# Visual-Behavior/detr-tensorflow

Measured on AMD Instinct MI355X. Metric: images/sec training step, DETR-R50 800x1333 bs=8/GPU, higher is better.
Workload: dtype bf16

## Files before the change

### detr-tensorflow_amd/csrc/conv_f32.hip

```cpp
#include "gemm_core.h"
#include "gemm_bf16_core.h"
#include "conv_args.h"
#include "conv_halo.h"
#include "conv_halo_dma.h"
namespace detr {

template <int BM, bool DGRAD, int DIL = 1>
struct LoaderConvA {
    static constexpr int NV = BM / 64;
    BufSrc src;
    int n_[NV], h_[NV], w_[NV];
    bool ok[NV];
    int kq, tid;

    __device__ __forceinline__ void init(const ConvArgs &a, int m0, int tid_) {
        src.init(a.src, (long long)a.N * a.Hs * a.Ws * a.Cs);
        tid = tid_;
        kq = (tid & 3) * 4;
#pragma unroll
        for (int i = 0; i < NV; ++i) {
            const int m = m0 + (tid >> 2) + 64 * i;
            ok[i] = m < a.M;
            const int mm = ok[i] ? m : 0;
            int wd, hd;
// ... 567 lines not shown
        if (++it_chunk == chunks) {
            it_chunk = 0;
            if (++it_ho == a.Ho) {
                it_ho = 0;
                ++it_n;
            }
        }
#pragma unroll
        for (int i = 0; i < NRD; ++i) {
            const int v = S16 ? 2 * tid : tid + 256 * i;
            const int j = 4 * (v >> 6) + ((v >> 2) & 3);
            const int col = 16 * ((v >> 4) & 3) + 4 * (v & 3);
            const bool ok = live && wo0 + j < a.Wo;
            const unsigned off = ((unsigned)((n * a.Ho + ho) * a.Wo + wo0 + j) * (unsigned)a.Co + (unsigned)(co0 + col)) * (S16 ? 2u : 4u);
            if constexpr (S16) rd[i] = ds.ld16(ok ? off : BUF_OOB);
            else rd[i] = ds.ld4(ok ? off : BUF_OOB);
        }
#pragma unroll
        for (int i = 0; i < NRX; ++i) {
            const int v = tid + 256 * i;
            const int pp = S16 ? v >> 3 : v >> 4, c4 = S16 ? 2 * (v & 7) : v & 15;
            const int kh = pp / PC, c = pp - kh * PC;
            const int hi = STR * ho - 1 + kh, wi = STR * wo0 - 1 + c;
            const bool ok = live && pp < NPP && hi >= 0 && hi < a.Hi && wi >= 0 && wi < a.Wi;
            const unsigned off = ((unsigned)((n * a.Hi + hi) * a.Wi + wi) * (unsigned)a.Ci + (unsigned)(ci0 + 4 * c4)) * (S16 ? 2u : 4u);
            if constexpr (S16) rx[i] = xs.ld16(ok ? off : BUF_OOB);
            else rx[i] = xs.ld4(ok ? off : BUF_OOB);
        }
    };
    auto store_unit = [&](int buf, const Reg (&rx)[NRX], const Reg (&rd)[NRD]) {
#pragma unroll
        for (int i = 0; i < NRD; ++i) {
            if constexpr (S16) *reinterpret_cast<uint4 *>(&sm.D[buf][tid * 8]) = rd[i];
            else *reinterpret_cast<uint2 *>(&sm.D[buf][(tid + 256 * i) * 4]) = make_uint2(pack_bf16(rd[i].x, rd[i].y), pack_bf16(rd[i].z, rd[i].w));
        }
#pragma unroll
        for (int i = 0; i < NRX; ++i) {
            const int v = tid + 256 * i;
            const int pp = S16 ? v >> 3 : v >> 4, c4 = S16 ? 2 * (v & 7) : v & 15;
            if (pp < NPP) {
                const int kh = pp / PC, c = WG::slot(pp - kh * PC);
                const int o = kh * WF_ROW + ((c >> 2) * 4 + (c4 >> 2)) * 64 + (((c & 3) + (c4 >> 2)) & 3) * 16 + (c4 & 3) * 4;
                if constexpr (S16) *reinterpret_cast<uint4 *>(&sm.X[buf][o]) = rx[i];
                else *reinterpret_cast<uint2 *>(&sm.X[buf][o]) = make_uint2(pack_bf16(rx[i].x, rx[i].y), pack_bf16(rx[i].z, rx[i].w));
            }
        }
    };
    typedef __attribute__((address_space(3))) s16x4 lds_s16x4;
    typedef short s16x8 __attribute__((ext_vector_type(8)));
    const int g = lane >> 4, t16 = lane & 15;
    int xo[2][3][2], dofs[2];
#pragma unroll
    for (int s2 = 0; s2 < 2; ++s2) {
        const int cib = 2 * wm + (g & 1);
        const int jbase = 16 * s2 + 8 * (g >> 1) + (t16 >> 2);
#pragma unroll
        for (int kw = 0; kw < 3; ++kw)
#pragma unroll
            for (int h = 0; h < 2; ++h) {
                const int c = STR == 1 ? jbase + kw + 4 * h : (kw & 1) * 33 + jbase + (kw >> 1) + 4 * h;
                xo[s2][kw][h] = ((c >> 2) * 4 + cib) * 64 + (((c & 3) + cib) & 3) * 16 + (t16 & 3) * 4;
            }
        dofs[s2] = ((4 * s2 + 2 * (g >> 1)) * 4 + 2 * wn + (g & 1)) * 64 + t16 * 4;
    }
    load_unit(u_begin, rx0, rd0);
    store_unit(0, rx0, rd0);
    load_unit(u_begin + 1, rx0, rd0);
    load_unit(u_begin + 2, rx1, rd1);
    lds_barrier();
    auto iter = [&](const int u, const int cur, Reg (&rpx)[NRX], Reg (&rpd)[NRD]) {
        store_unit(cur ^ 1, rpx, rpd);
        load_unit(u + 3, rpx, rpd);
        const unsigned short *X = sm.X[cur];
        const unsigned short *D = sm.D[cur];
#pragma unroll
        for (int s2 = 0; s2 < 2; ++s2) {
            const s16x4 blo = __builtin_amdgcn_ds_read_tr16_b64_v4i16((lds_s16x4 *)(D + dofs[s2]));
            const s16x4 bhi = __builtin_amdgcn_ds_read_tr16_b64_v4i16((lds_s16x4 *)(D + dofs[s2] + 4 * 64));
            const bf16x8 bfrag = __builtin_bit_cast(bf16x8, (s16x8)__builtin_shufflevector(blo, bhi, 0, 1, 2, 3, 4, 5, 6, 7));
#pragma unroll
            for (int kh = 0; kh < 3; ++kh)
#pragma unroll
                for (int kw = 0; kw < 3; ++kw) {
                    const s16x4 lo = __builtin_amdgcn_ds_read_tr16_b64_v4i16((lds_s16x4 *)(X + xo[s2][kw][0] + kh * WF_ROW));
                    const s16x4 hi = __builtin_amdgcn_ds_read_tr16_b64_v4i16((lds_s16x4 *)(X + xo[s2][kw][1] + kh * WF_ROW));
                    const bf16x8 afrag = __builtin_bit_cast(bf16x8, (s16x8)__builtin_shufflevector(lo, hi, 0, 1, 2, 3, 4, 5, 6, 7));
                    acc[kh * 3 + kw] = __builtin_amdgcn_mfma_f32_32x32x16_bf16(afrag, bfrag, acc[kh * 3 + kw], 0, 0, 0);
                }
        }
        lds_barrier();
    };
    {
        int u = u_begin;
        for (; u + 2 <= u_end; u += 2) {
            iter(u, 0, rx0, rd0);
            iter(u + 1, 1, rx1, rd1);
        }
        if (u < u_end) iter(u, 0, rx0, rd0);
    }
    if (a.slab_ts) {
#pragma unroll
        for (int t = 0; t < 9; ++t) {
            f32x16 one[1][1];
            one[0][0] = acc[t];
            float *slab = a.dw + (long long)blockIdx.z * a.part_stride + ((long long)(t * a.tiles_m + tm) * a.tiles_n + tn) * (64 * 64);
            store_slab_ts<64, 64, 2, 2>(one, slab, wave, lane);
        }
        return;
    }
    __syncthreads();
#pragma unroll
    for (int t = 0; t < 9; ++t) {
        f32x16 one[1][1];
        one[0][0] = acc[t];
        float *dw = a.dw + (long long)t * a.Ci * a.Co + (long long)blockIdx.z * a.part_stride;
        epilogue<64, 64, 2, 2, false>(one, reinterpret_cast<float *>(smem_raw), dw, a.Co, a.Ci, a.Co, ci0, co0, wm, wn, lane, wave, a.e, t == 0);
    }
}

typedef void (*ConvKernel)(ConvArgs);
typedef void (*WgradKernel)(ConvWgradArgs);

static void launch_conv_tiles(ConvKernel kernel, int bm, int bn, const ConvArgs &a0, hipStream_t s) {
    ConvArgs a = a0;
    a.tiles_m = cdiv(a.M, bm);
    a.tiles_n = cdiv(a.Cd, bn);
    dim3 grid((unsigned)(a.tiles_m * a.tiles_n)), block(GEMM_THREADS);
    hipLaunchKernelGGL(kernel, grid, block, 0, s, a);
}

template <int BM, int BN, int DIL, bool W16, bool X16>
static ConvKernel conv_bf16c_dir(bool dgrad) {
    return dgrad ? conv3x3_bf16c_kernel<BM, BN, 2, 2, true, W16, X16, DIL> : conv3x3_bf16c_kernel<BM, BN, 2, 2, false, W16, X16, DIL>;
}
template <int BM, int BN, int DIL>
static ConvKernel conv_bf16c_for(const ConvArgs &a, bool dgrad) {
    if (a.w16 && a.x16) return conv_bf16c_dir<BM, BN, DIL, true, true>(dgrad);
    if (a.w16) return conv_bf16c_dir<BM, BN, DIL, true, false>(dgrad);
    if (a.x16) return conv_bf16c_dir<BM, BN, DIL, false, true>(dgrad);
    return conv_bf16c_dir<BM, BN, DIL, false, false>(dgrad);
}

static bool x3_form(const ConvArgs &a) { return a.Cs % 32 == 0 && tune(T_X3_CONV) != 2 && (!a.par_on || tune(T_X3_CONV) == 1); }

template <int BM, int BN>
static void launch_conv(const ConvArgs &a, bool dgrad, hipStream_t s, bool split3 = false) {
    ConvKernel k = dgrad ? conv3x3_kernel<BM, BN, 2, 2, true> : conv3x3_kernel<BM, BN, 2, 2, false>;
    if constexpr (BM == BN) {
        if (split3 && x3_form(a)) k = dgrad ? conv3x3_x3_kernel<BM, BN, true> : conv3x3_x3_kernel<BM, BN, false>;
        else if (split3) k = dgrad ? conv3x3_kernel<BM, BN, 2, 2, true, true> : conv3x3_kernel<BM, BN, 2, 2, false, true>;
    }
    launch_conv_tiles(k, BM, BN, a, s);
}

static int wgrad_split_plan(int M, int tiles, int split, int &rps) {
    if (split <= 0) {
        split = cdiv(1536, tiles * 9);
        const int max_split = cdiv(M, 256);
        if (split > max_split) split = max_split;
        if (split < 1) split = 1;
    }
    rps = cdiv(M, split);
    rps = ((rps + BF_BK - 1) / BF_BK) * BF_BK;
    return cdiv(M, rps);
}
static int wgrad_x3_split(int M, int tiles, int bm) {
    const int rounds = tune(T_X3_WG_ROUNDS) > 0 ? tune(T_X3_WG_ROUNDS) : 2;
    const int slots = bm >= 128 ? 512 : 1024;
    int split = (rounds * slots) / (tiles * 9);
    const int max_split = cdiv(M, 256);
    if (split > max_split) split = max_split;
    return split < 1 ? 1 : split;
}
static int wgrad_fused_split_plan(int units, int tiles, int split, int &ups) {
    if (split <= 0) {
        int wgs = tune(T_WGRAD_FUSED_WGS);
        if (wgs <= 2) wgs = 512;
        split = cdiv(wgs, tiles);
    }
    if (split > units) split = units;
    if (split < 1) split = 1;
    ups = cdiv(units, split);
    return cdiv(units, ups);
}

struct WgradPlan {
    bool fused;
    int tile;
    int split;
    int per_split;
    long long bytes;
};

static WgradPlan wgrad_plan(int N, int Ho, int Wo, int Ci, int Co, int stride, int pad, bool s16, int compute, int dil, int split) {
    WgradPlan p;
    const bool bf = compute == 1 && Ci % 32 == 0 && Co % 32 == 0;
    const int fmode = tune(T_WGRAD_FUSED);
    const bool s_ok = stride == 1 || (stride == 2 && s16 && fmode != 3 && (fmode == 4 || (Ci <= 128 && Co <= 128)));
    p.fused = dil == 1 && bf && s_ok && pad == 1 && Ci % 64 == 0 && Co % 64 == 0 && fmode != 2;
    if (p.fused) {
        p.tile = 64;
        p.split = wgrad_fused_split_plan(N * Ho * cdiv(Wo, 32), (Ci / 64) * (Co / 64), split, p.per_split);
    } else {
        const int wforce = (bf || dil != 1) ? 0 : tune(T_WGRAD_TILE);
        p.tile = (wforce == 3) ? 64 : ((wforce == 1 || (Ci >= 128 && Co >= 128)) ? 128 : 64);
        const int M = N * Ho * Wo, tiles = cdiv(Ci, p.tile) * cdiv(Co, p.tile);
        if (compute == 2 && split <= 0 && tune(T_X3_CONV) != 2) split = wgrad_x3_split(M, tiles, p.tile);
        p.split = wgrad_split_plan(M, tiles, split, p.per_split);
    }
    p.bytes = p.split > 1 ? (long long)p.split * 9LL * Ci * Co * 4 : 0;
    return p;
}

template <class Launch>
static void wgrad_run(const ConvWgradArgs &a0, const WgradPlan &p, int taps_y, float *ws, long long ws_bytes, hipStream_t s, Launch launch) {
    ConvWgradArgs a = a0;
    a.tiles_m = cdiv(a.Ci, p.tile);
    a.tiles_n = cdiv(a.Co, p.tile);
    a.rows_per_split = p.per_split;
    const long long part = 9LL * a.Ci * a.Co;
    const bool partial = p.split > 1 && ws && aligned16(ws) && ws_bytes >= p.bytes;
    float *dw_final = a.dw;
    const EpiArgs final_e = a.e;
    a.part_stride = 0;
    a.slab_ts = 0;
    const bool ts = partial && a.Ci % p.tile == 0 && a.Co % p.tile == 0 && (!final_e.scale || aligned16(final_e.scale)) &&
                    aligned16(dw_final) && tune(T_SLAB_TS) != 2;
    if (partial) {
        a.dw = ws; a.part_stride = part;
        a.e.alpha = 1.0f;
        a.e.scale = nullptr;
        a.e.atomic = 0;
        a.e.vec = 1;
        a.slab_ts = ts ? 1 : 0;
    } else {
        a.e.atomic = 1;
    }
    launch(a, dim3((unsigned)(a.tiles_m * a.tiles_n), (unsigned)taps_y, (unsigned)p.split));
    if (partial) {
        detr_reduce_desc r = {};
        r.ws = ws; r.splits = p.split; r.part_stride = part; r.rows = 9 * a.Ci; r.cols = a.Co;
        r.C = dw_final; r.ldc = a.Co; r.alpha = final_e.alpha; r.scale = final_e.scale; r.rs_alpha = 1.0f;
        if (ts) { r.ts_bm = r.ts_bn = p.tile; r.ts_tiles_n = a.tiles_n; }
        launch_splitk_reduce(r, s);
    }
}

template <int BT>
static void launch_wgrad(const ConvWgradArgs &a0, const WgradPlan &p, float *ws, long long ws_bytes, hipStream_t s, bool bf16c, bool split3) {
    WgradKernel k;
    if (a0.dil == 2) {
        if (bf16c) k = a0.s16 ? conv3x3_wgrad_bf16c_kernel<BT, BT, 2, 2, true, 2> : conv3x3_wgrad_bf16c_kernel<BT, BT, 2, 2, false, 2>;
        else k = split3 ? conv3x3_wgrad_kernel<BT, BT, 2, 2, true, 2> : conv3x3_wgrad_kernel<BT, BT, 2, 2, false, 2>;
    } else if (bf16c) k = a0.s16 ? conv3x3_wgrad_bf16c_kernel<BT, BT, 2, 2, true> : conv3x3_wgrad_bf16c_kernel<BT, BT, 2, 2, false>;
    else if (split3) k = tune(T_X3_CONV) != 2 ? conv3x3_wgrad_x3_kernel<BT, BT> : conv3x3_wgrad_kernel<BT, BT, 2, 2, true>;
    else k = conv3x3_wgrad_kernel<BT, BT, 2, 2>;
    wgrad_run(a0, p, 9, ws, ws_bytes, s, [&](const ConvWgradArgs &a, dim3 grid) { hipLaunchKernelGGL(k, grid, dim3(GEMM_THREADS), 0, s, a); });
}

static void launch_wgrad_fused(const ConvWgradArgs &a0, const WgradPlan &p, float *ws, long long ws_bytes, hipStream_t s) {
    const int chunks = cdiv(a0.Wo, 32);
    wgrad_run(a0, p, 1, ws, ws_bytes, s, [&](const ConvWgradArgs &a, dim3 grid) {
        const dim3 block(GEMM_THREADS);
        if (a.stride == 2) hipLaunchKernelGGL((conv3x3_wgrad_fused_bf16_kernel<true, 2>), grid, block, 0, s, a, p.per_split, chunks);
        else if (a.s16) hipLaunchKernelGGL(conv3x3_wgrad_fused_bf16_kernel<true>, grid, block, 0, s, a, p.per_split, chunks);
        else hipLaunchKernelGGL(conv3x3_wgrad_fused_bf16_kernel<false>, grid, block, 0, s, a, p.per_split, chunks);
    });
}

static void launch_wgrad_plan(const ConvWgradArgs &a, const WgradPlan &p, float *ws, long long ws_bytes, hipStream_t s, bool bf16c, bool split3) {
    if (p.fused) launch_wgrad_fused(a, p, ws, ws_bytes, s);
    else if (p.tile == 128) launch_wgrad<128>(a, p, ws, ws_bytes, s, bf16c, split3);
    else launch_wgrad<64>(a, p, ws, ws_bytes, s, bf16c, split3);
}

void conv_dilated_tiles(const ConvArgs &a, bool dgrad, int compute, hipStream_t s) {
    ConvKernel k;
    if (compute == 1) k = conv_bf16c_for<64, 64, 2>(a, dgrad);
    else if (compute == 2) k = dgrad ? conv3x3_kernel<64, 64, 2, 2, true, true, 2> : conv3x3_kernel<64, 64, 2, 2, false, true, 2>;
    else k = dgrad ? conv3x3_kernel<64, 64, 2, 2, true, false, 2> : conv3x3_kernel<64, 64, 2, 2, false, false, 2>;
    launch_conv_tiles(k, 64, 64, a, s);
}

static WgradPlan conv_dilated_wgrad_plan(int N, int H, int W, int Ci, int Co, bool s16, int compute, int split) {
    return wgrad_plan(N, H, W, Ci, Co, 1, 2, s16, compute, 2, split);
}

void conv_dilated_wgrad_tiles(const ConvWgradArgs &a, int compute, int split, float *ws, long long ws_bytes, hipStream_t s) {
    launch_wgrad_plan(a, conv_dilated_wgrad_plan(a.N, a.Ho, a.Wo, a.Ci, a.Co, a.s16, compute, split), ws, ws_bytes, s, compute == 1, compute == 2);
}

int conv_dilated_wgrad_splits(int N, int H, int W, int Ci, int Co, int compute, int split) {
    return conv_dilated_wgrad_plan(N, H, W, Ci, Co, false, compute, split).split;
}

}

using namespace detr;

static WgradPlan wgrad_plan(const detr_conv3x3_desc *d) {
    return wgrad_plan(d->N, d->Ho, d->Wo, d->Ci, d->Co, d->stride, d->pad, d->x_dtype == 1 && d->w_dtype == 1, d->compute, 1, d->split);
}

static bool halo_eligible(const detr_conv3x3_desc *d, const ConvArgs &a, const EpiArgs &e, bool dgrad_classes) {
    if (!(d->compute == 1 && d->pad == 1 && a.w16 && a.x16 && e.c16 && a.Cs % 32 == 0 && a.Cd % 64 == 0 && a.Cd <= 512 &&
          (!d->mask || e.m16) && !d->residual && !d->scale && d->alpha == 1.0f && tune(T_CONV_HALO) != 2)) return false;
    if (dgrad_classes) return d->stride == 2 && !d->bias && d->act == 0 && tune(T_DGRAD_S2_CLASSES) != 3;
    return d->stride == 1 && (d->act == 0 || d->act == 1);
}

extern "C" int64_t detr_hip_workspace_bytes_conv3x3(const detr_conv3x3_desc *d, int32_t mode) {
    if (!d || d->N <= 0 || d->Ci <= 0 || d->Co <= 0) return -1;
    if (mode != 2) return 0;
    return wgrad_plan(d).bytes;
}

extern "C" int detr_hip_conv3x3_f32(const detr_conv3x3_desc *d, int32_t mode, void *stream) {
    DETR_REQUIRE(d != nullptr, "conv3x3: null descriptor");
    DETR_REQUIRE(mode >= 0 && mode <= 2, "conv3x3: bad mode %d", mode);
    DETR_REQUIRE(d->stride == 1 || d->stride == 2, "conv3x3: stride %d unsupported", d->stride);
    DETR_REQUIRE(d->Ci % 16 == 0 && d->Co % 16 == 0, "conv3x3: Ci=%d Co=%d must be multiples of 16", d->Ci, d->Co);
    DETR_REQUIRE(d->Ho == (d->Hi + 2 * d->pad - 3) / d->stride + 1 && d->Wo == (d->Wi + 2 * d->pad - 3) / d->stride + 1,
                 "conv3x3: output %dx%d inconsistent with input %dx%d pad %d stride %d", d->Ho, d->Wo, d->Hi, d->Wi,
                 d->pad, d->stride);
    DETR_REQUIRE(d->x && d->w && d->y, "conv3x3: null operand");
    DETR_REQUIRE(aligned16(d->x) && aligned16(d->w) && aligned16(d->y), "conv3x3: operands must be 16-byte aligned");
    DETR_REQUIRE((long long)d->N * d->Hi * d->Wi * d->Ci * 4 <= BUF_MAX_BYTES &&
                     (long long)d->N * d->Ho * d->Wo * d->Co * 4 <= BUF_MAX_BYTES,
                 "conv3x3: a tensor spans more than 4 GB (32-bit buffer offsets)");
    hipStream_t s = (hipStream_t)stream;
    EpiArgs e;
    e.alpha = d->alpha;
    e.scale = d->scale;
    e.bias = d->bias;
    e.residual = d->residual;
    e.mask = d->mask;
    e.act = d->act;
    e.atomic = 0;
    e.drop_scale = 0.0f; e.drop_thresh = 0; e.drop_seed = 0;
    const bool bits_in = d->mask && d->m_dtype == 2, bits_out = mode == 0 && d->maskbits_out != nullptr;
    e.vec = (!d->scale || aligned16(d->scale)) && (!d->bias || aligned16(d->bias)) &&
            (!d->residual || aligned16(d->residual)) && (!d->mask || bits_in || aligned16(d->mask));
    e.c16 = (mode != 2 && d->y_dtype == 1); e.r16 = d->r_dtype == 1;
    e.m16 = (d->m_dtype == 1 || d->m_dtype == 2) ? d->m_dtype : 0;
    if (mode == 2) {
        DETR_REQUIRE(!d->bias && !d->residual && !d->mask && d->act == 0, "conv3x3 wgrad: only scale/alpha epilogue");
        ConvWgradArgs a;
        a.N = d->N; a.Hi = d->Hi; a.Wi = d->Wi; a.Ci = d->Ci; a.Ho = d->Ho; a.Wo = d->Wo; a.Co = d->Co;
        a.stride = d->stride; a.pad = d->pad;
        a.x = d->x; a.dy = d->w; a.dw = d->y;
        a.M = d->N * d->Ho * d->Wo;
        a.s16 = (d->x_dtype == 1);
        DETR_REQUIRE(d->x_dtype == d->w_dtype && d->y_dtype == 0, "conv3x3 wgrad: x and dy must share their storage type, dw is fp32");
        DETR_REQUIRE(!a.s16 || (d->compute == 1 && d->Ci % 32 == 0 && d->Co % 32 == 0), "conv3x3 wgrad: bf16 tensors need compute = bf16");
        e.atomic = 1; e.ldr = 0; e.ldmask = 0;
        a.e = e;
        const bool bf = d->compute == 1 && d->Ci % 32 == 0 && d->Co % 32 == 0;
        const WgradPlan p = wgrad_plan(d);
        launch_wgrad_plan(a, p, d->workspace, d->workspace_bytes, s, bf, !bf && d->compute == 2);
        DETR_LAUNCH_CHECK(p.fused ? "conv3x3 wgrad bf16 (fused taps)" : (bf ? "conv3x3 wgrad bf16" : "conv3x3 wgrad"));
        return 0;
    }
    ConvArgs a;
    a.N = d->N; a.stride = d->stride; a.pad = d->pad; a.Ci = d->Ci; a.Co = d->Co;
    a.w = d->w; a.src = d->x; a.dst = d->y;
    if (mode == 0) {
        a.Hs = d->Hi; a.Ws = d->Wi; a.Cs = d->Ci;
        a.Hd = d->Ho; a.Wd = d->Wo; a.Cd = d->Co;
    } else {
        a.Hs = d->Ho; a.Ws = d->Wo; a.Cs = d->Co;
        a.Hd = d->Hi; a.Wd = d->Wi; a.Cd = d->Ci;
    }
    a.M = d->N * a.Hd * a.Wd;
    e.ldr = a.Cd;
    e.ldmask = bits_in ? a.Cd / 8 : a.Cd;
    e.mbits_out = bits_out ? d->maskbits_out : nullptr;
    e.ld_mbits_out = a.Cd / 8;
    e.wide16 = e.c16 && e.vec && (!d->residual || e.r16) && (!d->mask || e.m16) && (tune(T_EPI_WIDE) != 2 || bits_in || bits_out);
    DETR_REQUIRE(!(bits_in || bits_out) || (d->compute == 1 && e.wide16), "conv3x3: bit-packed masks need bf16 x / y / residual tensors (compute = bf16)");
    a.e = e;
    a.w16 = (d->w_dtype == 1);
    a.x16 = (d->x_dtype == 1);
    DETR_REQUIRE((d->x_dtype == 0 && d->y_dtype == 0 && d->r_dtype == 0 && d->m_dtype == 0) || (d->compute == 1 && d->Ci % 32 == 0 && d->Co % 32 == 0),
                 "conv3x3: bf16 tensors need compute = bf16 and channel counts %% 32 == 0");
    DETR_REQUIRE(d->w_dtype == 0 || (d->w_dtype == 1 && d->compute == 1 && mode != 2 && d->Ci % 32 == 0 && d->Co % 32 == 0),
                 "conv3x3: a bf16 kernel tensor needs compute = bf16, mode 0/1 and channel counts %% 32 == 0");
    a.par_on = 0; a.Hp = a.Wp = a.ph = a.pw = a.kh0 = a.kw0 = 0; a.nth = a.ntw = 3;
    a.cls_mix = 0;
    const bool dgrad = mode == 1;
    if (halo_eligible(d, a, e, false)) {
        if (a.Cd >= 128 && a.Cd % 128 == 0 && tune(T_CONV_DMA) != 2 && tune(T_CONV_HALO) != 4) { if (launch_conv_halo_dma(a, dgrad, s)) return -1; }
        else if (a.Cd % 128 == 0) { if (launch_conv_halo<128>(a, dgrad, s)) return -1; }
        else if (launch_conv_halo<64>(a, dgrad, s)) return -1;
        DETR_LAUNCH_CHECK("conv3x3 (halo)");
        return 0;
    }
    const int force = tune(T_CONV_TILE);
    auto launch = [&](const ConvArgs &c) {
        const long long big = (long long)cdiv(c.M, 128) * cdiv(c.Cd, 128);
        if (d->compute == 1 && c.Cs % 32 == 0 && c.Cd % 32 == 0) {
            if (force == 3 || (force == 0 && (c.Cd < 128 || big < 256)))
                launch_conv_tiles(conv_bf16c_for<64, 64, 1>(c, dgrad), 64, 64, c, s);
            else launch_conv_tiles(conv_bf16c_for<128, 128, 1>(c, dgrad), 128, 128, c, s);
        } else if (d->compute == 2) {
            const long long t192 = (long long)cdiv(c.M, 192) * cdiv(c.Cd, 128);
            const bool x3form = x3_form(c);
            if (force == 3 || (force == 0 && (c.Cd < 128 || big < x3_t128_threshold()))) launch_conv<64, 64>(c, dgrad, s, true);
            else if (force == 0 && x3form && tune(T_X3_T192) != 2 && tune(T_X3_T192) != 3 && (tune(T_X3_T192) == 1 || x3_t192_fewer_rounds(big, t192)))
                launch_conv_tiles(dgrad ? conv3x3_x3_kernel<192, 128, true> : conv3x3_x3_kernel<192, 128, false>, 192, 128, c, s);
            else if (force == 0 && x3form && tune(T_X3_T192) != 2 && (tune(T_X3_T192) == 3 || c.Cd == 128 || big <= 384)) 
                launch_conv_tiles(dgrad ? conv3x3_x3_kernel<128, 64, true> : conv3x3_x3_kernel<128, 64, false>, 128, 64, c, s);
            else launch_conv<128, 128>(c, dgrad, s, true);
        } else if (force == 1) launch_conv<128, 128>(c, dgrad, s);
        else if (force == 2) launch_conv<128, 64>(c, dgrad, s);
        else launch_conv<64, 64>(c, dgrad, s);
    };
    if (dgrad && d->stride == 2 && tune(T_DGRAD_S2_CLASSES) != 2) {
        if (halo_eligible(d, a, e, true)) {
            if (a.Cd % 128 == 0) { if (launch_conv_halo_s2classes<128>(a, s)) return -1; }
            else if (launch_conv_halo_s2classes<64>(a, s)) return -1;
            DETR_LAUNCH_CHECK("conv3x3 (halo, stride-2 classes)");
            return 0;
        }
        for (int ph = 0; ph < 2; ++ph)
            for (int pw = 0; pw < 2; ++pw) {
                ConvArgs c = a;
                c.par_on = 1; c.ph = ph; c.pw = pw;
                c.Hp = (a.Hd + 1 - ph) / 2;
                c.Wp = (a.Wd + 1 - pw) / 2;
                c.M = d->N * c.Hp * c.Wp;
                if (c.M <= 0) continue;
                c.kh0 = (ph + d->pad) & 1; c.kw0 = (pw + d->pad) & 1;
                c.nth = c.kh0 ? 1 : 2; c.ntw = c.kw0 ? 1 : 2;
                c.e.remap_w2 = c.Wp; c.e.remap_h2 = c.Hp; c.e.remap_W = a.Wd; c.e.remap_H = a.Hd;
                c.e.remap_ph = ph; c.e.remap_pw = pw;
                launch(c);
            }
    } else {
        launch(a);
    }
    DETR_LAUNCH_CHECK("conv3x3");
    return 0;
}
```

### detr-tensorflow_amd/csrc/conv_halo_dma.h

```cpp
#pragma once
#include "conv_halo.h"
#include "gemm_ring.h"

namespace detr {

constexpr int CHD_TH = 4, CHD_BN = 128, CHD_NB = 3;
constexpr int CHD_PIX = (CHD_TH + 2) * CH_PW;
constexpr int CHD_PP = (CHD_PIX + 15) / 16;
constexpr int CHD_PATCH = CHD_PP * 1024;
constexpr int CHD_BT = CHD_BN * BF_BK * 2;
constexpr int CHD_OFF_B = 2 * CHD_PATCH;
constexpr int CHD_OFF_DUMP = CHD_OFF_B + CHD_NB * CHD_BT;
constexpr int CHD_RING = CHD_OFF_DUMP + 1024;
constexpr int CHD_EPI = StageCfg<CHD_BN, 2>::BYTES;
constexpr int CHD_SMEM = CHD_RING > CHD_EPI ? CHD_RING : CHD_EPI;

template <bool DGRAD, bool LATE, bool DIL = false>
__global__ __launch_bounds__(GEMM_THREADS, 3) void conv3x3_halo_dma_bf16_kernel(ConvArgs a) {
#if defined(__HIP_DEVICE_COMPILE__)
    constexpr int BN = CHD_BN, TH = CHD_TH, NB = CHD_NB;
    using T = TileCfg<TH * CH_TW, BN, 2, 2>;
    extern __shared__ __attribute__((aligned(1024))) char chd_smem[];
    const int tid = threadIdx.x, lane = tid & 63;
    const int wave = __builtin_amdgcn_readfirstlane(tid >> 6);
    const int wm = wave >> 1, wn = wave & 1;
    int id = xcd_remap(blockIdx.x, gridDim.x);
    int ph = 0, pw = 0, Hp = a.Hp, Wp = a.Wp;
    if constexpr (DIL) halo_class_decode(a, id, ph, pw, Hp, Wp);
    const int tn = id % a.tiles_n;
    int t = id / a.tiles_n;
    const int twi = t % Wp;
    t /= Wp;
    const int thi = t % Hp;
    const int n = t / Hp;
    const int h0 = thi * TH, w0 = twi * CH_TW, n0 = tn * BN;
    const int nchunks = a.Cs / BF_BK;
    const unsigned lds0 = ring_lds_addr(chd_smem);

    const unsigned long long src_bytes = (unsigned long long)a.N * a.Hs * a.Ws * a.Cs * 2ull;
    unsigned pvoff[4];
    int plds[4];
#pragma unroll
    for (int i = 0; i < 4; ++i) {
        const int P = wave + 4 * i;
        const int px = 16 * P + (lane >> 2);
        const int pr = px / CH_PW, pc = px - pr * CH_PW;
        const int hq = h0 - 1 + pr, wq = w0 - 1 + pc;
        const int h = DIL ? 2 * hq + ph : hq, w = DIL ? 2 * wq + pw : wq;
        const int c = (lane & 3) ^ ((px >> 2) & 3);
        const bool ok = px < CHD_PIX && hq >= 0 && h < a.Hs && wq >= 0 && w < a.Ws;
        pvoff[i] = ok ? ((unsigned)((n * a.Hs + h) * a.Ws + w) * (unsigned)a.Cs) * 2u + 16u * (unsigned)c : BUF_OOB;
        plds[i] = P < CHD_PP ? P * 1024 : -1;
    }
    auto patch_issue = [&](const int i, const int c) {
        const unsigned left = (c < nchunks) ? (unsigned)(src_bytes - (unsigned long long)c * (BF_BK * 2)) : 0u;
        const u32x4 rs = ring_rsrc(reinterpret_cast<const char *>(a.src) + (long long)c * (BF_BK * 2), left);
        const int base = (c & 1) * CHD_PATCH;
        const int in = plds[i] >= 0 ? -1 : 0;
        const int off = CHD_OFF_DUMP + (in & (base + plds[i] - CHD_OFF_DUMP));
        ring_dma_piece(rs, lds0 + (unsigned)off, pvoff[i]);
    };
    const long long tapstride = (long long)a.Ci * a.Co;
    const unsigned long long w_bytes = 9ull * (unsigned long long)tapstride * 2ull;
    unsigned bvoff[2];
#pragma unroll
    for (int i = 0; i < 2; ++i) {
        const int P = wave + 4 * i;
        if constexpr (!DGRAD) {
            const int kr = lane >> 4, pc = lane & 15;
            const int col = n0 + 8 * (pc ^ (4 * kr));
            bvoff[i] = (col + 8 <= a.Cd) ? (unsigned)(4 * P + kr) * (unsigned)a.Co * 2u + 2u * (unsigned)col : BUF_OOB;
        } else {
            const int r = 16 * P + (lane >> 2);
            const int c = (lane & 3) ^ ((r >> 2) & 3);
            bvoff[i] = (n0 + r < a.Cd) ? (unsigned)(n0 + r) * (unsigned)a.Co * 2u + 16u * (unsigned)c : BUF_OOB;
        }
    }
    auto b_issue = [&](const int c, const int tp, const int slot) {
        const int wt = DGRAD ? 8 - tp : tp;
        const long long e0 = wt * tapstride + (DGRAD ? (long long)c * BF_BK : (long long)c * BF_BK * a.Co);
        const unsigned left = (c < nchunks) ? (unsigned)(w_bytes - (unsigned long long)e0 * 2ull) : 0u;
        const u32x4 rs = ring_rsrc(reinterpret_cast<const char *>(a.w) + e0 * 2, left);
#pragma unroll
        for (int i = 0; i < 2; ++i) ring_dma_piece(rs, lds0 + (unsigned)(CHD_OFF_B + slot * CHD_BT + (wave + 4 * i) * 1024), bvoff[i]);
    };

    f32x16 acc[T::TM][T::TN];
#pragma unroll
    for (int i = 0; i < T::TM; ++i)
#pragma unroll
        for (int j = 0; j < T::TN; ++j)
#pragma unroll
            for (int r = 0; r < 16; ++r) acc[i][j][r] = 0.0f;

    const int l31 = lane & 31, hh = lane >> 5;
    int p0[T::TM];
#pragma unroll
    for (int mi = 0; mi < T::TM; ++mi) p0[mi] = (HaloGeom<TH>::RB * wm + mi) * CH_PW + l31;
    int btr[T::TN], brow[T::TN];
#pragma unroll
    for (int ni = 0; ni < T::TN; ++ni) {
        btr[ni] = ring_tr_lane_off<1>(wn * T::WTN + ni * 32, lane);
        const int r = wn * T::WTN + ni * 32 + l31;
        brow[ni] = r * 64 + 16 * (hh ^ ((r >> 2) & 3));
    }
    bf16x8 fa[2][T::TM], fb[2][T::TN];
    auto read_tap = [&](const int pbuf, const int slot, const int tp) {
        const int toff = (tp / 3) * CH_PW + (tp - 3 * (tp / 3));
        const char *Pb = chd_smem + pbuf * CHD_PATCH;
        const char *Bs = chd_smem + CHD_OFF_B + slot * CHD_BT;
        int pa[T::TM];
#pragma unroll
        for (int mi = 0; mi < T::TM; ++mi) {
            int q = p0[mi];
            asm volatile("" : "+v"(q));
            const int p = q + toff;
            pa[mi] = p * 64 + 16 * (hh ^ ((p >> 2) & 3));
        }
#pragma unroll
        for (int kk = 0; kk < 2; ++kk) {
#pragma unroll
            for (int mi = 0; mi < T::TM; ++mi) fa[kk][mi] = *reinterpret_cast<const bf16x8 *>(Pb + (pa[mi] ^ (32 * kk)));
#pragma unroll
            for (int ni = 0; ni < T::TN; ++ni) {
                if constexpr (!DGRAD) fb[kk][ni] = ring_frag_tr<1>(Bs, btr[ni], kk);
                else fb[kk][ni] = *reinterpret_cast<const bf16x8 *>(Bs + (brow[ni] ^ (32 * kk)));
            }
        }
    };
    auto mma_half = [&](const int kk) {
#pragma unroll
        for (int mi = 0; mi < T::TM; ++mi)
#pragma unroll
            for (int ni = 0; ni < T::TN; ++ni) acc[mi][ni] = __builtin_amdgcn_mfma_f32_32x32x16_bf16(fa[kk][mi], fb[kk][ni], acc[mi][ni], 0, 0, 0);
    };

#pragma unroll
    for (int i = 0; i < 4; ++i) patch_issue(i, 0);
    b_issue(0, 0, 0);
    b_issue(0, 1, 1);
    for (int c = 0; c < nchunks; ++c) {
#pragma unroll
        for (int tp = 0; tp < 9; ++tp) {
            constexpr int READS = 2 * T::TM + (DGRAD ? 2 : 4) * T::TN, MF = 2 * T::TM * T::TN;
            if (tp >= 1 && tp <= 4) ring_wait_vmcnt<3>();
            else ring_wait_vmcnt<2>();
            __builtin_amdgcn_s_barrier();
            asm volatile("" ::: "memory");
            auto issue = [&]() {
                int cc = c;
                asm volatile("" : "+s"(cc));
                if (tp < 4) patch_issue(tp, cc + 1);
                b_issue(cc + (tp + 2) / 9, (tp + 2) % 9, (tp + 2) % NB);
            };
            if constexpr (!LATE) {
                issue();
                read_tap(c & 1, tp % NB, tp);
                mma_half(0);
                mma_half(1);
                sgb_ds_read<READS>();
                sgb_mfma_block<MF, 0, 0, 0>();
            } else {
                read_tap(c & 1, tp % NB, tp);
                mma_half(0);
                sgb_ds_read<READS>();
                sgb_mfma_block<MF / 2, 0, 0, 0>();
                __builtin_amdgcn_sched_barrier(0);
                issue();
                __builtin_amdgcn_sched_barrier(0);
                mma_half(1);
            }
            __builtin_amdgcn_sched_barrier(0);
        }
    }
    ring_wait_vmcnt<0>();
    __syncthreads();
    halo_epilogue<BN, TH, DIL>(acc, reinterpret_cast<float *>(chd_smem), reinterpret_cast<unsigned short *>(a.dst), a, n, h0, w0, n0, wm, wn, lane, wave, ph, pw);
#endif
}

static int launch_conv_halo_dma(const ConvArgs &a0, bool dgrad, hipStream_t s) {
    ConvArgs a = a0;
    a.Hp = cdiv(a.Hd, CHD_TH);
    a.Wp = cdiv(a.Wd, CH_TW);
    a.tiles_m = a.N * a.Hp * a.Wp;
    a.tiles_n = cdiv(a.Cd, CHD_BN);
    const bool late = tune(T_CONV_DMA) != 3;
    const int smem = CHD_SMEM;
    const int k = (dgrad ? 1 : 0) + (late ? 2 : 0);
    const void *fns[4] = {reinterpret_cast<const void *>(conv3x3_halo_dma_bf16_kernel<false, false>), reinterpret_cast<const void *>(conv3x3_halo_dma_bf16_kernel<true, false>),
                          reinterpret_cast<const void *>(conv3x3_halo_dma_bf16_kernel<false, true>), reinterpret_cast<const void *>(conv3x3_halo_dma_bf16_kernel<true, true>)};
    static bool reserved[4] = {false, false, false, false};
    if (!reserved[k]) {
        hipError_t err = hipFuncSetAttribute(fns[k], hipFuncAttributeMaxDynamicSharedMemorySize, smem);
        DETR_REQUIRE(err == hipSuccess, "conv3x3 (halo, DMA): cannot reserve %d bytes of LDS: %s", smem, hipGetErrorString(err));
        reserved[k] = true;
    }
    const dim3 grid((unsigned)(a.tiles_m * a.tiles_n)), block(GEMM_THREADS);
    switch (k) {
        case 0: hipLaunchKernelGGL((conv3x3_halo_dma_bf16_kernel<false, false>), grid, block, smem, s, a); break;
        case 1: hipLaunchKernelGGL((conv3x3_halo_dma_bf16_kernel<true, false>), grid, block, smem, s, a); break;
        case 2: hipLaunchKernelGGL((conv3x3_halo_dma_bf16_kernel<false, true>), grid, block, smem, s, a); break;
        default: hipLaunchKernelGGL((conv3x3_halo_dma_bf16_kernel<true, true>), grid, block, smem, s, a); break;
    }
    return 0;
}

static int launch_conv_halo_dma_planes(const ConvArgs &a0, bool dgrad, hipStream_t s) {
    ConvArgs a = a0;
    a.tiles_n = cdiv(a.Cd, CHD_BN);
    halo_class_plan(a, CHD_TH);
    if (a.cls_off[4] <= 0) return 0;
    a.cls_mix = 1;
    const int smem = CHD_SMEM;
    const void *fns[2] = {reinterpret_cast<const void *>(conv3x3_halo_dma_bf16_kernel<false, true, true>), reinterpret_cast<const void *>(conv3x3_halo_dma_bf16_kernel<true, true, true>)};
    static bool reserved[2] = {false, false};
    const int k = dgrad ? 1 : 0;
    if (!reserved[k]) {
        hipError_t err = hipFuncSetAttribute(fns[k], hipFuncAttributeMaxDynamicSharedMemorySize, smem);
        DETR_REQUIRE(err == hipSuccess, "conv3x3 dilated (halo planes, DMA): cannot reserve %d bytes of LDS: %s", smem, hipGetErrorString(err));
        reserved[k] = true;
    }
    const dim3 grid((unsigned)a.cls_off[4]), block(GEMM_THREADS);
    if (dgrad) hipLaunchKernelGGL((conv3x3_halo_dma_bf16_kernel<true, true, true>), grid, block, smem, s, a);
    else hipLaunchKernelGGL((conv3x3_halo_dma_bf16_kernel<false, true, true>), grid, block, smem, s, a);
    return 0;
}

}
```

Baseline: 531.0.

## Add stride-2 forward path to halo DMA conv via four parity-plane patch loads

Extends the DMA-fed halo conv3x3 kernel with a stride-2 forward variant. The input is split into four parity planes loaded into double-buffered LDS patches, and the nine taps are reordered so each plane buffer is reused across the taps that read it. Stride-2 bf16 forward convs in ResNet-50 with Cd%128==0 previously went through the generic implicit-GEMM tile kernel and now take this path. It adds a complex hand-scheduled tap/plane/vmcnt sequence that carries correctness risk, and it also folds the launch helpers into a single templated reserve-and-launch function.

Measured after the change: 533.4, median of 6. Within noise of the previous version (+0.5%).

```diff
diff --git a/detr-tensorflow_amd/csrc/conv_f32.hip b/detr-tensorflow_amd/csrc/conv_f32.hip
--- a/detr-tensorflow_amd/csrc/conv_f32.hip
+++ b/detr-tensorflow_amd/csrc/conv_f32.hip
@@ -893,11 +893,11 @@
     return wgrad_plan(d->N, d->Ho, d->Wo, d->Ci, d->Co, d->stride, d->pad, d->x_dtype == 1 && d->w_dtype == 1, d->compute, 1, d->split);
 }
 
-static bool halo_eligible(const detr_conv3x3_desc *d, const ConvArgs &a, const EpiArgs &e, bool dgrad_classes) {
+static bool halo_eligible(const detr_conv3x3_desc *d, const ConvArgs &a, const EpiArgs &e, bool dgrad_classes, int stride = 1) {
     if (!(d->compute == 1 && d->pad == 1 && a.w16 && a.x16 && e.c16 && a.Cs % 32 == 0 && a.Cd % 64 == 0 && a.Cd <= 512 &&
           (!d->mask || e.m16) && !d->residual && !d->scale && d->alpha == 1.0f && tune(T_CONV_HALO) != 2)) return false;
     if (dgrad_classes) return d->stride == 2 && !d->bias && d->act == 0 && tune(T_DGRAD_S2_CLASSES) != 3;
-    return d->stride == 1 && (d->act == 0 || d->act == 1);
+    return d->stride == stride && (d->act == 0 || d->act == 1);
 }
 
 extern "C" int64_t detr_hip_workspace_bytes_conv3x3(const detr_conv3x3_desc *d, int32_t mode) {
@@ -986,6 +986,11 @@
         DETR_LAUNCH_CHECK("conv3x3 (halo)");
         return 0;
     }
+    if (mode == 0 && halo_eligible(d, a, e, false, 2) && a.Cd % 128 == 0 && tune(T_CONV_DMA) != 2 && tune(T_CONV_DMA) != 4) {
+        if (launch_conv_halo_dma<true>(a, false, s)) return -1;
+        DETR_LAUNCH_CHECK("conv3x3 (halo, stride-2 plane steps)");
+        return 0;
+    }
     const int force = tune(T_CONV_TILE);
     auto launch = [&](const ConvArgs &c) {
         const long long big = (long long)cdiv(c.M, 128) * cdiv(c.Cd, 128);
diff --git a/detr-tensorflow_amd/csrc/conv_halo_dma.h b/detr-tensorflow_amd/csrc/conv_halo_dma.h
--- a/detr-tensorflow_amd/csrc/conv_halo_dma.h
+++ b/detr-tensorflow_amd/csrc/conv_halo_dma.h
@@ -4,21 +4,36 @@
 
 namespace detr {
 
-constexpr int CHD_TH = 4, CHD_BN = 128, CHD_NB = 3;
-constexpr int CHD_PIX = (CHD_TH + 2) * CH_PW;
-constexpr int CHD_PP = (CHD_PIX + 15) / 16;
-constexpr int CHD_PATCH = CHD_PP * 1024;
-constexpr int CHD_BT = CHD_BN * BF_BK * 2;
-constexpr int CHD_OFF_B = 2 * CHD_PATCH;
-constexpr int CHD_OFF_DUMP = CHD_OFF_B + CHD_NB * CHD_BT;
-constexpr int CHD_RING = CHD_OFF_DUMP + 1024;
-constexpr int CHD_EPI = StageCfg<CHD_BN, 2>::BYTES;
-constexpr int CHD_SMEM = CHD_RING > CHD_EPI ? CHD_RING : CHD_EPI;
-
-template <bool DGRAD, bool LATE, bool DIL = false>
+constexpr int CHD_TH = 4, CHD_BN = 128;
+template <bool S2 = false>
+struct HaloDmaCfg {
+    static constexpr int NB = 3;
+    static constexpr int PIX = (S2 ? CHD_TH + 1 : CHD_TH + 2) * CH_PW;
+    static constexpr int PP = (PIX + 15) / 16;
+    static constexpr int NPW = (PP + 3) / 4;
+    static constexpr int PATCH = PP * 1024;
+    static constexpr int BT = CHD_BN * BF_BK * 2;
+    static constexpr int OFF_B = 2 * PATCH;
+    static constexpr int OFF_DUMP = OFF_B + NB * BT;
+    static constexpr int RING = OFF_DUMP + 1024;
+    static constexpr int EPI = StageCfg<CHD_BN, 2>::BYTES;
+    static constexpr int SMEM = RING > EPI ? RING : EPI;
+};
+
+__host__ __device__ constexpr int chd_s2_plane(int tp) { return tp == 2 ? 3 : (tp < 5 ? 0 : (tp < 7 ? 1 : 2)); }
+__host__ __device__ constexpr int chd_s2_buf(int tp) { return (tp == 2 || tp == 5 || tp == 6) ? 1 : 0; }
+__host__ __device__ constexpr int chd_s2_tap(int tp) { return tp == 0 ? 0 : tp == 1 ? 2 : tp == 2 ? 4 : tp == 3 ? 6 : tp == 4 ? 8 : tp == 5 ? 1 : tp == 6 ? 7 : tp == 7 ? 3 : 5; }
+__host__ __device__ constexpr int chd_s2_off(int tp) { return tp == 0 ? 0 : (tp == 1 || tp == 5) ? 1 : (tp == 3 || tp == 7) ? 3 : 4; }
+__host__ __device__ constexpr int chd_s2_req_plane(int tp) { return tp == 0 ? 3 : tp == 3 ? 1 : tp == 5 ? 2 : tp == 7 ? 0 : -1; }
+__host__ __device__ constexpr int chd_s2_req_buf(int tp) { return tp == 5 ? 0 : 1; }
+__host__ __device__ constexpr int chd_s2_keep(int tp) { return (tp == 1 || tp == 4 || tp == 6 || tp == 8) ? 3 : 0; }
+
+template <bool DGRAD, bool LATE, bool DIL = false, bool S2 = false>
 __global__ __launch_bounds__(GEMM_THREADS, 3) void conv3x3_halo_dma_bf16_kernel(ConvArgs a) {
+    static_assert(!S2 || (!DGRAD && !DIL), "the stride-2 plane steps exist for the forward");
 #if defined(__HIP_DEVICE_COMPILE__)
-    constexpr int BN = CHD_BN, TH = CHD_TH, NB = CHD_NB;
+    using C = HaloDmaCfg<S2>;
+    constexpr int BN = CHD_BN, TH = CHD_TH, NB = C::NB, NPW = C::NPW, NBP = 2;
     using T = TileCfg<TH * CH_TW, BN, 2, 2>;
     extern __shared__ __attribute__((aligned(1024))) char chd_smem[];
     const int tid = threadIdx.x, lane = tid & 63;
@@ -37,34 +52,40 @@
     const int nchunks = a.Cs / BF_BK;
     const unsigned lds0 = ring_lds_addr(chd_smem);
 
+    constexpr int NPL = S2 ? 4 : 1;
     const unsigned long long src_bytes = (unsigned long long)a.N * a.Hs * a.Ws * a.Cs * 2ull;
-    unsigned pvoff[4];
-    int plds[4];
-#pragma unroll
-    for (int i = 0; i < 4; ++i) {
+    unsigned pvoff[NPL][NPW];
+    int plds[NPW];
+#pragma unroll
+    for (int i = 0; i < NPW; ++i) {
         const int P = wave + 4 * i;
         const int px = 16 * P + (lane >> 2);
         const int pr = px / CH_PW, pc = px - pr * CH_PW;
         const int hq = h0 - 1 + pr, wq = w0 - 1 + pc;
-        const int h = DIL ? 2 * hq + ph : hq, w = DIL ? 2 * wq + pw : wq;
         const int c = (lane & 3) ^ ((px >> 2) & 3);
-        const bool ok = px < CHD_PIX && hq >= 0 && h < a.Hs && wq >= 0 && w < a.Ws;
-        pvoff[i] = ok ? ((unsigned)((n * a.Hs + h) * a.Ws + w) * (unsigned)a.Cs) * 2u + 16u * (unsigned)c : BUF_OOB;
-        plds[i] = P < CHD_PP ? P * 1024 : -1;
-    }
-    auto patch_issue = [&](const int i, const int c) {
+#pragma unroll
+        for (int k = 0; k < NPL; ++k) {
+            const int py = S2 ? (k < 2 ? 1 : 0) : ph, pxp = S2 ? ((k & 1) ? 0 : 1) : pw;
+            const int h = (DIL || S2) ? 2 * hq + py : hq, w = (DIL || S2) ? 2 * wq + pxp : wq;
+            const bool read = !S2 || ((py == 1 || pr >= 1) && (pxp == 1 || pc >= 1));
+            const bool ok = px < C::PIX && hq >= 0 && h < a.Hs && wq >= 0 && w < a.Ws && read;
+            pvoff[k][i] = ok ? ((unsigned)((n * a.Hs + h) * a.Ws + w) * (unsigned)a.Cs) * 2u + 16u * (unsigned)c : BUF_OOB;
+        }
+        plds[i] = P < C::PP ? P * 1024 : -1;
+    }
+    auto patch_issue = [&](const int i, const int k, const int c, const int buf) {
         const unsigned left = (c < nchunks) ? (unsigned)(src_bytes - (unsigned long long)c * (BF_BK * 2)) : 0u;
         const u32x4 rs = ring_rsrc(reinterpret_cast<const char *>(a.src) + (long long)c * (BF_BK * 2), left);
-        const int base = (c & 1) * CHD_PATCH;
+        const int base = buf * C::PATCH;
         const int in = plds[i] >= 0 ? -1 : 0;
-        const int off = CHD_OFF_DUMP + (in & (base + plds[i] - CHD_OFF_DUMP));
-        ring_dma_piece(rs, lds0 + (unsigned)off, pvoff[i]);
+        const int off = C::OFF_DUMP + (in & (base + plds[i] - C::OFF_DUMP));
+        ring_dma_piece(rs, lds0 + (unsigned)off, pvoff[k][i]);
     };
     const long long tapstride = (long long)a.Ci * a.Co;
     const unsigned long long w_bytes = 9ull * (unsigned long long)tapstride * 2ull;
-    unsigned bvoff[2];
-#pragma unroll
-    for (int i = 0; i < 2; ++i) {
+    unsigned bvoff[NBP];
+#pragma unroll
+    for (int i = 0; i < NBP; ++i) {
         const int P = wave + 4 * i;
         if constexpr (!DGRAD) {
             const int kr = lane >> 4, pc = lane & 15;
@@ -77,12 +98,12 @@
         }
     }
     auto b_issue = [&](const int c, const int tp, const int slot) {
-        const int wt = DGRAD ? 8 - tp : tp;
+        const int wt = S2 ? chd_s2_tap(tp) : (DGRAD ? 8 - tp : tp);
         const long long e0 = wt * tapstride + (DGRAD ? (long long)c * BF_BK : (long long)c * BF_BK * a.Co);
         const unsigned left = (c < nchunks) ? (unsigned)(w_bytes - (unsigned long long)e0 * 2ull) : 0u;
         const u32x4 rs = ring_rsrc(reinterpret_cast<const char *>(a.w) + e0 * 2, left);
 #pragma unroll
-        for (int i = 0; i < 2; ++i) ring_dma_piece(rs, lds0 + (unsigned)(CHD_OFF_B + slot * CHD_BT + (wave + 4 * i) * 1024), bvoff[i]);
+        for (int i = 0; i < NBP; ++i) ring_dma_piece(rs, lds0 + (unsigned)(C::OFF_B + slot * C::BT + (wave + 4 * i) * 1024), bvoff[i]);
     };
 
     f32x16 acc[T::TM][T::TN];
@@ -107,8 +128,8 @@
     bf16x8 fa[2][T::TM], fb[2][T::TN];
     auto read_tap = [&](const int pbuf, const int slot, const int tp) {
         const int toff = (tp / 3) * CH_PW + (tp - 3 * (tp / 3));
-        const char *Pb = chd_smem + pbuf * CHD_PATCH;
-        const char *Bs = chd_smem + CHD_OFF_B + slot * CHD_BT;
+        const char *Pb = chd_smem + pbuf * C::PATCH;
+        const char *Bs = chd_smem + C::OFF_B + slot * C::BT;
         int pa[T::TM];
 #pragma unroll
         for (int mi = 0; mi < T::TM; ++mi) {
@@ -136,32 +157,42 @@
     };
 
 #pragma unroll
-    for (int i = 0; i < 4; ++i) patch_issue(i, 0);
+    for (int i = 0; i < NPW; ++i) patch_issue(i, 0, 0, 0);
     b_issue(0, 0, 0);
     b_issue(0, 1, 1);
     for (int c = 0; c < nchunks; ++c) {
 #pragma unroll
         for (int tp = 0; tp < 9; ++tp) {
             constexpr int READS = 2 * T::TM + (DGRAD ? 2 : 4) * T::TN, MF = 2 * T::TM * T::TN;
-            if (tp >= 1 && tp <= 4) ring_wait_vmcnt<3>();
-            else ring_wait_vmcnt<2>();
+            const int keep = S2 ? chd_s2_keep(tp) : ((tp >= 1 && tp <= NPW) ? 1 : 0);
+            if (keep == 0) ring_wait_vmcnt<NBP>();
+            else if (keep == 1) ring_wait_vmcnt<NBP + 1>();
+            else ring_wait_vmcnt<NBP + 3>();
             __builtin_amdgcn_s_barrier();
             asm volatile("" ::: "memory");
             auto issue = [&]() {
                 int cc = c;
                 asm volatile("" : "+s"(cc));
-                if (tp < 4) patch_issue(tp, cc + 1);
+                if constexpr (S2) {
+                    if (chd_s2_req_plane(tp) >= 0) {
+#pragma unroll
+                        for (int i = 0; i < NPW; ++i) patch_issue(i, chd_s2_req_plane(tp), cc + (tp == 7 ? 1 : 0), (cc & 1) ^ chd_s2_req_buf(tp));
+                    }
+                } else {
+                    if (tp < NPW) patch_issue(tp, 0, cc + 1, (cc + 1) & 1);
+                }
                 b_issue(cc + (tp + 2) / 9, (tp + 2) % 9, (tp + 2) % NB);
             };
+            const int pbuf = S2 ? ((c & 1) ^ chd_s2_buf(tp)) : (c & 1), poff = S2 ? chd_s2_off(tp) : tp;
             if constexpr (!LATE) {
                 issue();
-                read_tap(c & 1, tp % NB, tp);
+                read_tap(pbuf, tp % NB, poff);
                 mma_half(0);
                 mma_half(1);
                 sgb_ds_read<READS>();
                 sgb_mfma_block<MF, 0, 0, 0>();
             } else {
-                read_tap(c & 1, tp % NB, tp);
+                read_tap(pbuf, tp % NB, poff);
                 mma_half(0);
                 sgb_ds_read<READS>();
                 sgb_mfma_block<MF / 2, 0, 0, 0>();
@@ -179,31 +210,35 @@
 #endif
 }
 
+template <bool DGRAD, bool LATE, bool DIL = false, bool S2 = false>
+static int launch_conv_halo_dma_kernel(const ConvArgs &a, unsigned grid, hipStream_t s) {
+    constexpr int smem = HaloDmaCfg<S2>::SMEM;
+    static bool reserved = false;
+    if (!reserved) {
+        hipError_t err = hipFuncSetAttribute(reinterpret_cast<const void *>(conv3x3_halo_dma_bf16_kernel<DGRAD, LATE, DIL, S2>), hipFuncAttributeMaxDynamicSharedMemorySize, smem);
+        DETR_REQUIRE(err == hipSuccess, "conv3x3 (halo, DMA): cannot reserve %d bytes of LDS: %s", smem, hipGetErrorString(err));
+        reserved = true;
+    }
+    hipLaunchKernelGGL((conv3x3_halo_dma_bf16_kernel<DGRAD, LATE, DIL, S2>), dim3(grid), dim3(GEMM_THREADS), smem, s, a);
+    return 0;
+}
+
+template <bool S2 = false>
 static int launch_conv_halo_dma(const ConvArgs &a0, bool dgrad, hipStream_t s) {
     ConvArgs a = a0;
+    DETR_REQUIRE(a.Cd % CHD_BN == 0, "conv3x3 (halo, DMA): %d output channels are not whole %d-channel tiles (the epilogue has no column guard)", a.Cd, CHD_BN);
     a.Hp = cdiv(a.Hd, CHD_TH);
     a.Wp = cdiv(a.Wd, CH_TW);
     a.tiles_m = a.N * a.Hp * a.Wp;
     a.tiles_n = cdiv(a.Cd, CHD_BN);
-    const bool late = tune(T_CONV_DMA) != 3;
-    const int smem = CHD_SMEM;
-    const int k = (dgrad ? 1 : 0) + (late ? 2 : 0);
-    const void *fns[4] = {reinterpret_cast<const void *>(conv3x3_halo_dma_bf16_kernel<false, false>), reinterpret_cast<const void *>(conv3x3_halo_dma_bf16_kernel<true, false>),
-                          reinterpret_cast<const void *>(conv3x3_halo_dma_bf16_kernel<false, true>), reinterpret_cast<const void *>(conv3x3_halo_dma_bf16_kernel<true, true>)};
-    static bool reserved[4] = {false, false, false, false};
-    if (!reserved[k]) {
-        hipError_t err = hipFuncSetAttribute(fns[k], hipFuncAttributeMaxDynamicSharedMemorySize, smem);
-        DETR_REQUIRE(err == hipSuccess, "conv3x3 (halo, DMA): cannot reserve %d bytes of LDS: %s", smem, hipGetErrorString(err));
-        reserved[k] = true;
-    }
-    const dim3 grid((unsigned)(a.tiles_m * a.tiles_n)), block(GEMM_THREADS);
-    switch (k) {
-        case 0: hipLaunchKernelGGL((conv3x3_halo_dma_bf16_kernel<false, false>), grid, block, smem, s, a); break;
-        case 1: hipLaunchKernelGGL((conv3x3_halo_dma_bf16_kernel<true, false>), grid, block, smem, s, a); break;
-        case 2: hipLaunchKernelGGL((conv3x3_halo_dma_bf16_kernel<false, true>), grid, block, smem, s, a); break;
-        default: hipLaunchKernelGGL((conv3x3_halo_dma_bf16_kernel<true, true>), grid, block, smem, s, a); break;
-    }
-    return 0;
+    const unsigned grid = (unsigned)(a.tiles_m * a.tiles_n);
+    if constexpr (S2) {
+        DETR_REQUIRE(!dgrad, "conv3x3 (halo, DMA): the stride-2 plane steps are a forward kernel");
+        return launch_conv_halo_dma_kernel<false, true, false, true>(a, grid, s);
+    } else {
+        if (tune(T_CONV_DMA) == 3) return dgrad ? launch_conv_halo_dma_kernel<true, false>(a, grid, s) : launch_conv_halo_dma_kernel<false, false>(a, grid, s);
+        return dgrad ? launch_conv_halo_dma_kernel<true, true>(a, grid, s) : launch_conv_halo_dma_kernel<false, true>(a, grid, s);
+    }
 }
 
 static int launch_conv_halo_dma_planes(const ConvArgs &a0, bool dgrad, hipStream_t s) {
@@ -212,19 +247,8 @@
     halo_class_plan(a, CHD_TH);
     if (a.cls_off[4] <= 0) return 0;
     a.cls_mix = 1;
-    const int smem = CHD_SMEM;
-    const void *fns[2] = {reinterpret_cast<const void *>(conv3x3_halo_dma_bf16_kernel<false, true, true>), reinterpret_cast<const void *>(conv3x3_halo_dma_bf16_kernel<true, true, true>)};
-    static bool reserved[2] = {false, false};
-    const int k = dgrad ? 1 : 0;
-    if (!reserved[k]) {
-        hipError_t err = hipFuncSetAttribute(fns[k], hipFuncAttributeMaxDynamicSharedMemorySize, smem);
-        DETR_REQUIRE(err == hipSuccess, "conv3x3 dilated (halo planes, DMA): cannot reserve %d bytes of LDS: %s", smem, hipGetErrorString(err));
-        reserved[k] = true;
-    }
-    const dim3 grid((unsigned)a.cls_off[4]), block(GEMM_THREADS);
-    if (dgrad) hipLaunchKernelGGL((conv3x3_halo_dma_bf16_kernel<true, true, true>), grid, block, smem, s, a);
-    else hipLaunchKernelGGL((conv3x3_halo_dma_bf16_kernel<false, true, true>), grid, block, smem, s, a);
-    return 0;
-}
-
-}
+    const unsigned grid = (unsigned)a.cls_off[4];
+    return dgrad ? launch_conv_halo_dma_kernel<true, true, true>(a, grid, s) : launch_conv_halo_dma_kernel<false, true, true>(a, grid, s);
+}
+
+}
```
